# nadongjun/mirbft

Hardware: AMD Instinct MI355X
Metric: SHA-256 digests/s (request + batch digests), Actions.Hash stream (higher is better)
Workload: dtype u32

## Files before the change

### mirbft_amd/csrc/mirsha_api.hip

```cpp
#include "mirsha_ctx.h"

namespace mirsha_api {

int fail(mirsha_ctx* c, int code, const char* fmt, ...) {
    char buf[512];
    va_list ap;
    va_start(ap, fmt);
    vsnprintf(buf, sizeof(buf), fmt, ap);
    va_end(ap);
    if (c) c->err = buf;
    return code;
}

hipEvent_t take_event(KernelTimer& t) {
    if (!t.pool.empty()) {
        hipEvent_t e = t.pool.back();
        t.pool.pop_back();
        return e;
    }
    hipEvent_t e = nullptr;
    if (hipEventCreate(&e) != hipSuccess) return nullptr;
    return e;
}

// ... 81 lines not shown

int queue_bucket_order(mirsha_ctx* c, const OrderShape& sh, const uint32_t* d_len, uint32_t n, uint32_t* d_order) {
    uint32_t* counts = c->d_order_counts.as<uint32_t>();
    const size_t cells = (size_t)sh.bins * sh.n_chunks;
    uint32_t* base = counts + cells;
    if (int rc = timed_launch(c, kTimerOrder, [&] {
            return mirsha::launch_order_count(d_len, n, sh.bmax, sh.bins, sh.chunk, sh.n_chunks, counts, c->stream);
        }))
        return rc;
    size_t scan_bytes = sh.scan_bytes;
    HIP_TRY(c, mirsha::launch_counts_scan(c->d_scan.p, scan_bytes, counts, base, cells, c->stream));
    return timed_launch(c, kTimerOrder, [&] {
        return mirsha::launch_order_scatter(d_len, n, sh.bmax, sh.bins, sh.chunk, sh.n_chunks, base, d_order,
                                            c->stream);
    });
}

}

extern "C" {

int mirsha_version(void) { return (0 << 16) | 2; }

int mirsha_device_count(int* count) {
    if (!count) return MIRSHA_EINVAL;
    int n = 0;
    if (hipGetDeviceCount(&n) != hipSuccess) {
        (void)hipGetLastError();
        n = 0;
    }
    *count = n;
    return MIRSHA_OK;
}

int mirsha_ctx_create(int device, mirsha_ctx** out) {
    if (!out) return MIRSHA_EINVAL;
    *out = nullptr;
    int n = 0;
    if (hipGetDeviceCount(&n) != hipSuccess || n <= 0) {
        (void)hipGetLastError();
        return MIRSHA_ENODEV;
    }
    if (device < 0 || device >= n) return MIRSHA_EINVAL;
    hipDeviceProp_t prop;
    if (hipGetDeviceProperties(&prop, device) != hipSuccess) return MIRSHA_EHIP;
    if (strncmp(prop.gcnArchName, "gfx950", 6) != 0) return MIRSHA_ENODEV;
    mirsha_ctx* c = new mirsha_ctx();
    c->device = device;
    if (hipSetDevice(device) != hipSuccess || hipStreamCreateWithFlags(&c->own, hipStreamNonBlocking) != hipSuccess) {
        delete c;
        return MIRSHA_EHIP;
    }
    c->stream = c->own;
    *out = c;
    return MIRSHA_OK;
}

void mirsha_ctx_destroy(mirsha_ctx* c) {
    if (!c) return;
    (void)hipSetDevice(c->device);
    (void)hipStreamSynchronize(c->stream);
    if (c->xin) (void)hipStreamSynchronize(c->xin);
    if (c->xout) (void)hipStreamSynchronize(c->xout);
    if (c->xcommit) (void)hipStreamSynchronize(c->xcommit);
    for (auto& t : c->timers) {
        for (auto& pr : t.pending) { (void)hipEventDestroy(pr.first); (void)hipEventDestroy(pr.second); }
        for (auto e : t.pool) (void)hipEventDestroy(e);
    }
    c->d_arena.release(); c->d_off.release(); c->d_len.release(); c->d_order.release();
    c->d_out.release(); c->d_idx.release(); c->d_first.release(); c->d_out2.release(); c->d_scratch.release();
    c->d_scan.release();
    c->d_order_counts.release();
    for (int k = 0; k < kStageSlots; k++) {
        c->h_ring[k].release();
        if (c->ring_ev[k]) (void)hipEventDestroy(c->ring_ev[k]);
    }
    c->h_meta.release();
    c->h_outs.release();
    c->d_meta.release();
    c->h_expect.release(); c->h_verdict.release(); c->d_expect.release(); c->d_verdict.release();
    for (auto e : c->xev) (void)hipEventDestroy(e);
    if (c->xin) (void)hipStreamDestroy(c->xin);
    if (c->xout) (void)hipStreamDestroy(c->xout);
    if (c->xcommit) (void)hipStreamDestroy(c->xcommit);
    for (auto& sl : c->slots) {
        sl.stage.release(); sl.dig.release(); sl.dev.release(); sl.stage2.release(); sl.dev2.release();
        sl.xp.stage.release(); sl.xp.verdict.release(); sl.xp.dev.release();
        sl.cm.stage.release(); sl.cm.dev.release(); sl.cm.snap.release(); sl.cm.rows.release();
        if (sl.done) (void)hipEventDestroy(sl.done);
        if (sl.ev_in) (void)hipEventDestroy(sl.ev_in);
        if (sl.ev_kern) (void)hipEventDestroy(sl.ev_kern);
    }
    if (c->own) (void)hipStreamDestroy(c->own);
    delete c;
}

const char* mirsha_last_error(const mirsha_ctx* c) { return c ? c->err.c_str() : "null context"; }

int mirsha_ctx_set_stream(mirsha_ctx* c, void* s) {
    if (!c) return MIRSHA_EINVAL;
    c->stream = s ? static_cast<hipStream_t>(s) : c->own;
    return MIRSHA_OK;
}

void* mirsha_ctx_stream(mirsha_ctx* c) { return c ? static_cast<void*>(c->stream) : nullptr; }

int mirsha_ctx_set_variant(mirsha_ctx* c, int v) {
    if (!c || !mirsha::variant_valid(v)) return MIRSHA_EINVAL;
    c->variant = v;
    return MIRSHA_OK;
}

int mirsha_ctx_set_timing(mirsha_ctx* c, int enable) {
    if (!c) return MIRSHA_EINVAL;
    c->timing = enable != 0;
    return MIRSHA_OK;
}

int mirsha_ctx_kernel_time(mirsha_ctx* c, int which, uint64_t* launches, double* total_ms) {
    if (!c || which < 0 || which >= kKernelTimers) return MIRSHA_EINVAL;
    if (int rc = use_device(c)) return rc;
    KernelTimer& t = c->timers[which];
    for (auto& pr : t.pending) {
        HIP_TRY(c, hipEventSynchronize(pr.second));
// ... 237 lines not shown
```

### mirbft_amd/csrc/mirsha_ctx.h

```cpp
#pragma once
#include <hip/hip_runtime.h>

#include <algorithm>
#include <atomic>
#include <chrono>
#include <condition_variable>
#include <cstdarg>
#include <cstdio>
#include <cstdlib>
#include <cstring>
#include <functional>
#include <mutex>
#include <string>
#include <thread>
#include <vector>

#include "../../include/mirsha.h"
#include "mirsha_host.h"
#include "mirsha_device.h"
#include "mirsha_order.h"
#include "mirsha_sha512.h"
#include "mirsha_sha512_pair.h"
#include "mirsha_sha512_plan.h"

// ... 107 lines not shown
    uint8_t* out = nullptr;
    uint32_t n = 0;
    uint64_t* bits = nullptr;
    uint32_t* count = nullptr;
};

struct AsyncSlot {
    PinnedBuf stage;
    Clock::time_point t_queued;
    PinnedBuf dig;
    DevBuf dev;
    PinnedBuf stage2;
    DevBuf dev2;
    hipEvent_t done = nullptr;
    hipEvent_t ev_in = nullptr, ev_kern = nullptr;
    uint64_t ticket = 0;
    bool busy = false;
    SlotRetire retire;
    std::vector<uint32_t> rank;
    double prof[MIRSHA_PROF_PHASES] = {};
    ExpectSlot xp;
    CommitSlot cm;
};

constexpr int kKernelTimers = 10;
constexpr int kTimerVerify = 6;
constexpr int kTimerExpect = 7;
constexpr int kTimerOrder = 8;
constexpr int kTimerStreams = 9;

struct KernelTimer {
    std::vector<std::pair<hipEvent_t, hipEvent_t>> pending;
    std::vector<hipEvent_t> pool;
    uint64_t launches = 0;
    double ms = 0.0;
};


}
using namespace mirsha_api;

struct mirsha_ctx {
    int device = 0;
    hipStream_t own = nullptr;
    hipStream_t stream = nullptr;
    int variant = mirsha::kVariantLds;
    int hasher = MIRSHA_HASHER_SHA256;
    mutable uint64_t sha512_pair_launches = 0;
    bool timing = false;
    uint32_t time_mask = 0xFFFFFFFFu;
    std::string err;
    DevBuf d_arena, d_off, d_len, d_order, d_out, d_idx, d_first, d_out2, d_scratch;
    DevBuf d_scan;
    int order_mode = MIRSHA_ORDER_HOST;
    DevBuf d_order_counts;
    PinnedBuf h_ring[kStageSlots];
    hipEvent_t ring_ev[kStageSlots] = {};
    bool ring_busy[kStageSlots] = {};
    PinnedBuf h_meta, h_outs;
    DevBuf d_meta;
    hipStream_t xin = nullptr, xout = nullptr;
    std::vector<hipEvent_t> xev;
    std::vector<uint32_t> sl_len;
    std::vector<uint64_t> sl_poff;
    KernelTimer timers[kKernelTimers];
    PinnedBuf h_expect, h_verdict;
    DevBuf d_expect, d_verdict;
    AsyncSlot slots[kAsyncSlots];
    std::vector<uint64_t> xp_has;
    std::vector<uint32_t> xp_base;
    hipStream_t xcommit = nullptr;
    std::vector<uint32_t> cm_plan;
    uint64_t next_ticket = 1;
    uint64_t done_ticket = 0;
    double prof[MIRSHA_PROF_PHASES] = {};
};

struct RingOwner {
    hipEvent_t ev = nullptr;
    bool queued = false;
};

struct mirsha_chains {
    int device = 0;
    uint32_t n = 0;
    int hasher = MIRSHA_HASHER_SHA256;
    DevBuf d_h, d_pend, d_cnt;
    DevBuf d_dig, d_pos, d_act, d_afirst, d_which, d_out;
    std::vector<uint32_t> plan;
    DevBuf d_plan;
    RingOwner ring;
    uint64_t pair_launches = 0;
};

struct mirsha_streams {
    int device = 0;
    uint32_t n = 0;
    int hasher = MIRSHA_HASHER_SHA256;
    uint32_t row_bytes = 0;
    DevBuf d_state;
    std::vector<uint32_t> act, efirst, kind, len;
    std::vector<uint64_t> off, poff;
    std::vector<uint32_t> seg_stream, sfirst, seg_flags;
    PinnedBuf stage;
    DevBuf dev, d_out;
    RingOwner ring;
// ... 22 lines not shown
    DevBuf d_seg_nb, d_seg_state, d_seg_flags;
    uint64_t seg_runs = 0;
    int fallback = 0;
    uint32_t test_placement = 0;
    DevBuf d_probe;
    bool trace = false;
    std::vector<uint32_t> cidx, cfirst;
    uint32_t uniform = 0;
    std::vector<uint32_t> order;
    DevBuf d_cidx, d_cfirst, d_order;
};

namespace mirsha_api {

int fail(mirsha_ctx* c, int code, const char* fmt, ...);

#define HIP_TRY(c, expr)                                                                    \
    do {                                                                                    \
        hipError_t _e = (expr);                                                             \
        if (_e != hipSuccess)                                                               \
            return fail((c), _e == hipErrorOutOfMemory ? MIRSHA_ENOMEM : MIRSHA_EHIP,       \
                        "%s: %s (%s:%d)", #expr, hipGetErrorString(_e), __FILE__, __LINE__); \
    } while (0)

hipEvent_t take_event(KernelTimer& t);

template <class F>
int timed_launch(mirsha_ctx* c, int which, F&& launch) {
    hipEvent_t e0 = nullptr, e1 = nullptr;
    const bool timed = c->timing && ((c->time_mask >> which) & 1u);
    if (timed) {
        e0 = take_event(c->timers[which]);
        e1 = take_event(c->timers[which]);
        if (e0 && e1) mirsha::next_launch_events() = {e0, e1};
    }
    hipError_t e = launch();
    const bool bound = e0 && e1 && !mirsha::next_launch_events().start;
    mirsha::next_launch_events() = {};
    if (timed && (!bound || e != hipSuccess)) {
        if (e0) c->timers[which].pool.push_back(e0);
        if (e1) c->timers[which].pool.push_back(e1);
    }
    if (e != hipSuccess) return fail(c, MIRSHA_EHIP, "kernel launch: %s", hipGetErrorString(e));
    if (bound) c->timers[which].pending.emplace_back(e0, e1);
    return MIRSHA_OK;
}

inline hipError_t hasher_launch_msgs(const mirsha_ctx* c, const uint8_t* arena, uint64_t arena_len,
                                     const uint64_t* off, const uint32_t* len, const uint32_t* order, uint32_t n,
                                     uint8_t* out, hipStream_t s) {
    if (c->hasher == MIRSHA_HASHER_SHA512_256)
        return mirsha::launch_sha512_msgs(arena, arena_len, off, len, order, n, out, c->variant, s,
                                          &c->sha512_pair_launches);
    return mirsha::launch_msgs(arena, arena_len, off, len, order, n, out, c->variant, s);
}
inline hipError_t hasher_launch_lists(const mirsha_ctx* c, const uint8_t* digests, uint32_t n_digests,
                                      const uint32_t* idx, uint32_t n_entries, const uint32_t* first, uint32_t n_lists,
                                      uint32_t* scratch, uint8_t* out, hipStream_t s) {
    if (c->hasher == MIRSHA_HASHER_SHA512_256)
        return mirsha::launch_sha512_lists(digests, n_digests, idx, n_entries, first, n_lists, scratch, out, s,
                                           &c->sha512_pair_launches);
    return mirsha::launch_lists(digests, n_digests, idx, n_entries, first, n_lists, scratch, out, s);
}

inline const char* hasher_name(int hasher) { return hasher == MIRSHA_HASHER_SHA512_256 ? "sha512_256" : "sha256"; }

inline int sha256_only(mirsha_ctx* c, const char* call) {
    if (!c || c->hasher == MIRSHA_HASHER_SHA256) return MIRSHA_OK;
    return fail(c, MIRSHA_EINVAL, "%s: hasher %s is not built for this call", call, hasher_name(c->hasher));
}

inline int chains_hasher_match(mirsha_ctx* c, const mirsha_chains* ch, const char* call) {
    if (!c || !ch || c->hasher == ch->hasher) return MIRSHA_OK;
    return fail(c, MIRSHA_EINVAL, "%s: the chains hash with %s, the context with %s", call, hasher_name(ch->hasher),
                hasher_name(c->hasher));
}

inline int plan_hasher_match(mirsha_ctx* c, const mirsha_pipeline* p, const char* call) {
    if (!c || !p || c->hasher == p->hasher) return MIRSHA_OK;
    return fail(c, MIRSHA_EINVAL, "%s: the plan hashes with %s, the context with %s", call, hasher_name(p->hasher),
                hasher_name(c->hasher));
}

inline int streams_hasher_match(mirsha_ctx* c, const mirsha_streams* st, const char* call) {
    if (!c || !st || c->hasher == st->hasher) return MIRSHA_OK;
    return fail(c, MIRSHA_EINVAL, "%s: the streams hash with %s, the context with %s", call, hasher_name(st->hasher),
                hasher_name(c->hasher));
}

int use_device(mirsha_ctx* c);

inline uint32_t host_blocks(uint32_t L) { return (uint32_t)(((uint64_t)L + 72u) >> 6); }

bool bucket_order(const uint32_t* len, uint32_t n, uint32_t* order);

struct OrderShape {
    uint32_t bmax = 0, bins = 0, chunk = 0, n_chunks = 0;
    size_t scan_bytes = 0;
};
int order_buffers(mirsha_ctx* c, uint32_t n, uint32_t bmin, uint32_t bmax, OrderShape* shape);
int queue_bucket_order(mirsha_ctx* c, const OrderShape& shape, const uint32_t* d_len, uint32_t n, uint32_t* d_order);

inline int owner_order(mirsha_ctx* c, const RingOwner& o) {
    if (!o.queued) return MIRSHA_OK;
    HIP_TRY(c, hipStreamWaitEvent(c->stream, o.ev, 0));
    return MIRSHA_OK;
}
// ... 210 lines not shown
```

### mirbft_amd/csrc/mirsha_kernels.h

```cpp
#pragma once
#include <hip/hip_runtime.h>
#include <stdint.h>

namespace mirsha {

constexpr uint32_t kWavesPerBlock = 4;
constexpr uint32_t kBlockThreads = 64 * kWavesPerBlock;
constexpr uint32_t kNullIndex = 0xFFFFFFFFu;

enum : int {
    kVariantLds = 0,
    kVariantDirect = 1,
    kVariantLowOcc = 4,
    kVariantLdsOnly = 5,
    kVariantPair = 6,
    kVariantCu = 10,
};
const char* ab_getenv(const char* name);
inline bool variant_valid(int v) {
    return v == kVariantLds || v == kVariantDirect || v == kVariantLowOcc || v == kVariantLdsOnly || v == kVariantPair ||
           v == kVariantCu;
}
constexpr uint32_t kCuMaxWavesPerSimd = 4;
uint32_t cu_count();
constexpr uint32_t kLowOccTiles = 1024;
constexpr uint32_t kPairMaxGroups = 512;
uint32_t pair_max_groups();

constexpr uint64_t kMaxBufferArena = 0xFFFFFF00ull;
constexpr uint32_t kMaxBufferMsgs = 1u << 27;
hipError_t launch_offsets_scan(void* tmp, size_t& tmp_bytes, const uint32_t* len, uint64_t* off, uint32_t n,
                               hipStream_t s);
struct LaunchEvents {
    hipEvent_t start = nullptr, stop = nullptr;
};
LaunchEvents& next_launch_events();

hipError_t launch_msgs(const uint8_t* arena, uint64_t arena_len, const uint64_t* off,
                       const uint32_t* len, const uint32_t* order, uint32_t n, uint8_t* out,
                       int variant, hipStream_t s);
constexpr uint32_t kMaxListDigests = (1u << 27) - 1u;
constexpr uint32_t kMaxListEntries = (1u << 30) - 1u;
hipError_t launch_lists(const uint8_t* digests, uint32_t n_digests, const uint32_t* idx, uint32_t n_entries,
                        const uint32_t* first, uint32_t n_lists, uint32_t* scratch, uint8_t* out, hipStream_t s);
struct PadBlockKW {
    uint32_t kw[64];
    uint32_t use;
};
PadBlockKW pad_block_kw(uint64_t L);
hipError_t launch_chain(const uint8_t* digests, uint32_t n_digests, const uint32_t* cidx, uint32_t n_entries,
                        const uint32_t* cfirst, uint32_t n_lists, uint8_t* out, hipStream_t s, uint32_t uniform = 0);
hipError_t launch_chain_pair(const uint8_t* digests, uint32_t n_digests, const uint32_t* cidx, uint32_t n_entries,
                             const uint32_t* cfirst, uint32_t n_lists, uint8_t* out, hipStream_t s);
struct OverlapArgs {
    const uint8_t* arena;
    uint64_t arena_len;
    const uint64_t* off;
    const uint32_t* len;
    const uint32_t* order;
    uint32_t n_req;
    uint8_t* req_out;
    const uint8_t* prev_digests;
    uint32_t n_req_prev;
    const uint32_t* cidx;
    uint32_t n_entries;
    const uint32_t* cfirst;
    uint32_t n_lists;
    uint8_t* list_out;
    uint32_t list_waves;
    uint32_t chain_prio;
};
hipError_t launch_msgs_overlap(const OverlapArgs& a, hipStream_t s);
constexpr uint32_t kFusedChunkBlocks = 2;
constexpr uint32_t kFusedMaxQueues = 4;
constexpr uint32_t kCtlTileTicket = 0, kCtlDone = 80, kCtlWords = 96;
constexpr unsigned long long kFusedWatchdogTicks = 200000000ull;
struct FusedArgs {
    const uint8_t* arena;
    const uint64_t* off;
    const uint32_t* len;
    const uint32_t* order;
    uint8_t* req_out;
    const uint32_t* cidx;
    const uint32_t* cfirst;
    uint8_t* list_out;
    const uint32_t* tadj_first;
    const uint32_t* tadj;
    const uint32_t* cbase;
    const uint32_t* expected;
    unsigned long long* counters;
    unsigned long long* ctl;
    unsigned long long* err;
    unsigned long long watchdog;
// ... 43 lines not shown
```

### mirbft_amd/csrc/mirsha_kernels.hip

```cpp
#include <algorithm>
#include <atomic>
#include <cstdlib>
#include <cstdio>
#include <type_traits>

#include "mirsha_device.h"

namespace mirsha {

struct RawChunk {
    uint32_t v[5];
    uint32_t sel;
};

__device__ __forceinline__ void issue_chunk(__amdgpu_buffer_rsrc_t rsrc, uint32_t records, uint32_t o,
                                            uint32_t blk, uint32_t q, bool active, RawChunk& c) {
    const uint32_t addr = o + 64u * blk + 16u * q;
    const uint32_t a = active ? (addr & ~3u) : 0xFFFFFFE0u;
    c.sel = be_sel(addr & 3u);
    if (a + 20u <= records || !active) {
        const auto v = __builtin_amdgcn_raw_buffer_load_b128(rsrc, a, 0, 0);
        c.v[0] = v[0]; c.v[1] = v[1]; c.v[2] = v[2]; c.v[3] = v[3];
        c.v[4] = __builtin_amdgcn_raw_buffer_load_b32(rsrc, a + 16u, 0, 0);
    } else {
// ... 161 lines not shown
__device__ __forceinline__ void balance_done() {
    __hip_atomic_store(g_bal_prog + bal_word(), kBalDone, __ATOMIC_RELAXED, __HIP_MEMORY_SCOPE_WORKGROUP);
}

__device__ __forceinline__ void wave_lds_handoff() {
    __builtin_amdgcn_fence(__ATOMIC_RELEASE, "wavefront");
    __builtin_amdgcn_wave_barrier();
    __builtin_amdgcn_fence(__ATOMIC_ACQUIRE, "wavefront");
}

__device__ __forceinline__ void tile_read_words(const uint4* tile, uint32_t lane, uint32_t w[16]) {
#pragma unroll
    for (int k = 0; k < 4; k++) {
        const uint4 x = tile[lds_slot(lane, (uint32_t)k)];
        w[4 * k + 0] = x.x; w[4 * k + 1] = x.y; w[4 * k + 2] = x.z; w[4 * k + 3] = x.w;
    }
}

__device__ __forceinline__ bool last_block_opaque(uint32_t wave_nb, uint32_t blk) {
    uint32_t wnb;
    asm volatile("s_mov_b32 %0, %1" : "=s"(wnb) : "s"(wave_nb));
    return wnb - blk == 1u;
}

template <bool kFused, bool kBuf>
__device__ __forceinline__ void tile_store(uint8_t* out, uint32_t n, uint32_t msg, const uint32_t st[8]) {
    if constexpr (kFused || kBuf) {
        const __amdgpu_buffer_rsrc_t ors =
            __builtin_amdgcn_make_buffer_rsrc((void*)out, (short)0, (int)(32u * n), 0x00020000);
        if constexpr (kFused)
            store_digest_sc1(ors, msg, st);
        else
            store_digest_buf(ors, msg, st);
    } else {
        store_digest(out, msg, st);
    }
}

template <bool kFused>
__device__ __forceinline__ void block_prio(uint32_t fprio, uint32_t blk) {
    if constexpr (kFused) {
        if (fprio == kPrioBalance)
            balance_prio(blk);
        else if (fprio == kPrioProgress)
            progress_prio(blk);
        else
            fixed_prio(fprio);
    } else {
        progress_prio(blk);
    }
}

constexpr uint32_t kTilePaused = 0, kTileDone = 1;
template <bool kLds, bool kWide, bool kFused = false, bool kDma = false>
__device__ __forceinline__ uint32_t hash_tile(const uint8_t* __restrict__ arena, uint64_t arena_len,
                                          const uint64_t* __restrict__ off, const uint32_t* __restrict__ len,
                                          const uint32_t* __restrict__ order, uint32_t n, uint8_t* __restrict__ out,
                                          uint4* my, uint32_t t, uint32_t lane, uint32_t fprio = 0,
                                          uint32_t b0 = 0u, uint32_t b1 = 0xFFFFFFFFu, uint32_t* st_io = nullptr,
                                          uint32_t lone_sel = 0u, uint4* my2 = nullptr,
                                          unsigned long long* lone_tr = nullptr) {
    __builtin_amdgcn_s_setprio(3);
    const uint32_t slot = t * 64u + lane;
    const bool valid = slot < n;
    const uint32_t slot_c = valid ? slot : n - 1u;
    const uint32_t msg = order ? order[slot_c] : slot_c;
    const uint32_t L_ = len[msg];
    const uint64_t o_ = off[msg];
    const uint32_t L = valid ? L_ : 0u;
    const uint64_t o = valid ? o_ : 0u;
    const uint32_t nb = valid ? blocks_for_len(L) : 0u;
    const uint32_t max_l = wave_max(valid ? L : 0u);
    const uint32_t wave_nb = blocks_for_len(max_l);

    const uint64_t records = (arena_len + 3u) & ~3ull;
    const __amdgpu_buffer_rsrc_t rsrc =
        __builtin_amdgcn_make_buffer_rsrc((void*)arena, (short)0, (int)(uint32_t)records, 0x00020000);
    auto issue = [&](uint64_t mo, uint32_t blk, uint32_t q, bool active, RawChunk& rc) {
        if constexpr (kWide)
            issue_chunk_wide(arena, records, mo, blk, q, active, rc);
        else
            issue_chunk(rsrc, (uint32_t)records, (uint32_t)mo, blk, q, active, rc);
    };

    uint32_t st[8];
#pragma unroll
    for (int i = 0; i < 8; i++) st[i] = (st_io && b0) ? st_io[i] : kH0[i];
    const bool finished = b1 >= wave_nb;

    if constexpr (kLds && !kWide) {
        const uint32_t q = lane & 3u;
        const uint64_t reach = valid ? o + 64ull * wave_nb + 20u : 0ull;
        const bool far = __builtin_amdgcn_ballot_w64(reach > records) == 0;
        const bool aligned = __builtin_amdgcn_ballot_w64(valid && (o & 3u) != 0u) == 0;
        const uint32_t min_l = wave_min(valid ? L : 0xFFFFFFFFu);
        const bool uni = max_l == min_l;
        const int32_t u_last = (int32_t)(min_l - 64u * (wave_nb - 1u));
        const bool tail_ok = uni && u_last <= 16;
        const TailWords tw = tail_words(u_last, min_l);
        uint32_t vo[4], sel[4];
#pragma unroll
        for (int j = 0; j < 4; j++) {
            const uint32_t a = (uint32_t)__shfl((int)(uint32_t)o, 16 * j + (int)(lane >> 2), 64) + 16u * q;
            vo[j] = a & ~3u;
            sel[j] = be_sel(a & 3u);
        }
        auto stage = [&](uint32_t blk, uint32_t w[16], uint32_t ln, bool trim) {
            const uint32_t soff = 64u * blk;
            const uint32_t qq = ln & 3u;
            const bool skip = trim && soff + 16u * qq >= min_l;
            RawChunk rc[4];
            if (far && !trim) {
#pragma unroll
                for (int j = 0; j < 4; j++) {
                    const auto v = __builtin_amdgcn_raw_buffer_load_b128(rsrc, vo[j], soff, 0);
                    rc[j].v[0] = v[0]; rc[j].v[1] = v[1]; rc[j].v[2] = v[2]; rc[j].v[3] = v[3];
                    rc[j].v[4] = 0u;
                }
                if (!aligned) {
#pragma unroll
                    for (int j = 0; j < 4; j++)
                        rc[j].v[4] = __builtin_amdgcn_raw_buffer_load_b32(rsrc, vo[j], soff + 16u, 0);
                }
            } else if (far) {
#pragma unroll
                for (int j = 0; j < 4; j++) {
                    const uint32_t a = skip ? 0xFFFFFFE0u : vo[j] + soff;
                    const auto v = __builtin_amdgcn_raw_buffer_load_b128(rsrc, a, 0, 0);
                    rc[j].v[0] = v[0]; rc[j].v[1] = v[1]; rc[j].v[2] = v[2]; rc[j].v[3] = v[3];
                    rc[j].v[4] = aligned ? 0u : __builtin_amdgcn_raw_buffer_load_b32(rsrc, a + 16u, 0, 0);
                }
            } else {
#pragma unroll
                for (int j = 0; j < 4; j++)
                    issue_chunk(rsrc, (uint32_t)records, vo[j] + soff, 0u, 0u, !skip, rc[j]);
            }
            const bool pad = soff + 64u > min_l;
#pragma unroll
            for (int j = 0; j < 4; j++) {
                uint32_t wq[4];
#pragma unroll
                for (int k = 0; k < 4; k++) wq[k] = be_word(rc[j].v[k + 1], rc[j].v[k], sel[j]);
                if (pad && !uni) {
                    const uint32_t Lm = (uint32_t)__shfl((int)L, 16 * j + (int)(ln >> 2), 64);
                    pad_words(soff + 16u * qq, Lm, blk + 1u == blocks_for_len(Lm), qq, wq);
                }
                my[lds_slot(16u * j + (ln >> 2), qq)] = make_uint4(wq[0], wq[1], wq[2], wq[3]);
            }
            wave_lds_handoff();
            tile_read_words(my, ln, w);
            wave_lds_handoff();
        };
// ... 33 lines not shown
                uint32_t w[16];
                const uint4* tb = tile_of(blk);
#pragma unroll
                for (int k = 0; k < 4; k++) {
                    const uint4 x = tb[lds_slot(lane, (uint32_t)k)];
                    w[4 * k + 0] = x.x; w[4 * k + 1] = x.y; w[4 * k + 2] = x.z; w[4 * k + 3] = x.w;
                }
                asm volatile("s_waitcnt lgkmcnt(0)" ::: "memory");
                if (blk + (deep ? 2u : 1u) < d1) issue_dma(blk + (deep ? 2u : 1u));
#pragma unroll
                for (int k = 0; k < 16; k++) w[k] = __builtin_bswap32(w[k]);
                if (soff + 64u > dmin) {
                    const bool last = last_block_opaque(wave_nb, blk);
                    if (uni) {
                        pad_block_uniform(w, soff, dmin, last);
                    } else {
#pragma unroll
                        for (int k = 0; k < 4; k++)
                            pad_words(soff + 16u * (uint32_t)k, L, blk + 1u == nb, (uint32_t)k, &w[4 * k]);
                    }
                }
                if constexpr (!kFused) block_prio<false>(fprio, blk);
                if constexpr (kFused) {
                    if (lone_sel != 0u && simd_alone(lone_sel)) lone_sel = kLoneSeen;
                    if (lone_sel == kLoneSeen) {
                        if (lone_tr != nullptr) {
                            if (lane == 0u) *lone_tr |= 1ull << 63 | (unsigned long long)min(blk, 1023u) << 53;
                            lone_tr = nullptr;
                        }
                        if (blk < nb) compress_asm_lat(st, w);
                    } else if (blk < nb) {
                        compress_asm(st, w);
                    }
                } else if (blk < nb) {
                    compress_asm(st, w);
                }
            }
        }
        for (uint32_t blk = dma ? loop_end : b0; blk < loop_end; blk++) {
            const uint32_t soff = 64u * blk;
            uint32_t w[16];
            stage(blk, w, lane, false);
            if (soff + 64u > min_l && uni)
                pad_block_uniform(w, soff, min_l, last_block_opaque(wave_nb, blk));
            block_prio<kFused>(fprio, blk);
            if (blk < nb) compress_asm(st, w);
        }
        if (tail_ok && finished) {
            const uint32_t blk = wave_nb - 1u;
            uint32_t w[16];
            uint32_t ln;
            asm volatile("v_mov_b32 %0, %1" : "=v"(ln) : "v"(lane));
            stage(blk, w, ln, true);
            pad_block_uniform<4>(w, 64u * blk, min_l, false);
            block_prio<kFused>(fprio, blk);
            if (blk < nb) compress_asm_tail(st, w, tw);
        }
    } else if constexpr (kLds) {
        const uint32_t q = lane & 3u;
        uint32_t Lj[4], nbj[4];
        uint64_t oj[4];
#pragma unroll
        for (int j = 0; j < 4; j++) {
            const int src = 16 * j + (int)(lane >> 2);
            Lj[j] = (uint32_t)__shfl((int)L, src, 64);
            oj[j] = (uint64_t)(uint32_t)__shfl((int)(uint32_t)o, src, 64);
            oj[j] |= (uint64_t)(uint32_t)__shfl((int)(uint32_t)(o >> 32), src, 64) << 32;
            nbj[j] = (uint32_t)__shfl((int)nb, src, 64);
        }
        for (uint32_t blk = 0; blk < wave_nb; blk++) {
            RawChunk rc[4];
#pragma unroll
            for (int j = 0; j < 4; j++) issue(oj[j], blk, q, blk < nbj[j], rc[j]);
#pragma unroll
            for (int j = 0; j < 4; j++) {
                uint32_t wq[4];
                finish_chunk(rc[j], 64u * blk + 16u * q, Lj[j], blk + 1u == nbj[j], q, wq);
                my[lds_slot(16u * j + (lane >> 2), q)] = make_uint4(wq[0], wq[1], wq[2], wq[3]);
            }
            wave_lds_handoff();
            uint32_t w[16];
#pragma unroll
            for (int k = 0; k < 4; k++) {
                const uint4 x = my[lds_slot(lane, (uint32_t)k)];
                w[4 * k + 0] = x.x; w[4 * k + 1] = x.y; w[4 * k + 2] = x.z; w[4 * k + 3] = x.w;
            }
            wave_lds_handoff();
            progress_prio(blk);
            if (blk < nb) compress_asm(st, w);
        }
    } else {
        for (uint32_t blk = 0; blk < wave_nb; blk++) {
            const bool active = blk < nb;
            RawChunk rc[4];
#pragma unroll
            for (int q = 0; q < 4; q++) issue(o, blk, (uint32_t)q, active, rc[q]);
            uint32_t w[16];
#pragma unroll
            for (int q = 0; q < 4; q++)
                finish_chunk(rc[q], 64u * blk + 16u * q, L, blk + 1u == nb, (uint32_t)q, &w[4 * q]);
            progress_prio(blk);
            if (active) compress_asm(st, w);
        }
    }
    if (!finished) {
#pragma unroll
        for (int i = 0; i < 8; i++) st_io[i] = st[i];
        return kTilePaused;
    }
    if (valid) tile_store<kFused, kLds && !kWide>(out, n, msg, st);
    return kTileDone;
}

constexpr uint32_t kMsgWaves = 1;
constexpr uint32_t kMsgOcc = 8, kTileSlots = 256;
template <bool kLds, bool kWide = false>
__global__ __launch_bounds__(64 * kMsgWaves, kWide ? 6 : kMsgOcc) void sha256_msgs_kernel(
    const uint8_t* __restrict__ arena, uint64_t arena_len, const uint64_t* __restrict__ off,
    const uint32_t* __restrict__ len, const uint32_t* __restrict__ order, uint32_t n,
    uint8_t* __restrict__ out) {
    __shared__ uint4 tile[kMsgWaves][kTileSlots];
    const uint32_t lane = threadIdx.x & 63u;
    const uint32_t wv = threadIdx.x >> 6;
    const uint32_t t = blockIdx.x * kMsgWaves + wv;
    if (t * 64u >= n) return;
    hash_tile<kLds, kWide>(arena, arena_len, off, len, order, n, out, tile[wv], t, lane);
}

constexpr uint32_t kCuLds = 96u * 1024u;
__global__ __launch_bounds__(1024, 1) void sha256_msgs_cu_kernel(const uint8_t* __restrict__ arena,
                                                                 uint64_t arena_len,
                                                                 const uint64_t* __restrict__ off,
                                                                 const uint32_t* __restrict__ len,
                                                                 const uint32_t* __restrict__ order, uint32_t n,
                                                                 uint8_t* __restrict__ out) {
    extern __shared__ uint4 cu_lds[];
    const uint32_t lane = threadIdx.x & 63u;
    const uint32_t wv = threadIdx.x >> 6;
    const uint32_t t = blockIdx.x * (blockDim.x >> 6) + wv;
    if (t * 64u >= n) return;
    hash_tile<true, false, false, true>(arena, arena_len, off, len, order, n, out, cu_lds + 256u * wv, t, lane);
}

__device__ __forceinline__ void overlap_chain(const uint8_t* __restrict__ digests, uint32_t n_digests,
                                              const uint32_t* __restrict__ cidx, uint32_t n_entries,
                                              const uint32_t* __restrict__ cfirst, uint32_t n_lists,
                                              uint8_t* __restrict__ list_out, uint32_t g, uint32_t lane,
                                              uint32_t prio_mode) {
    __builtin_amdgcn_s_setprio(3);
    const uint32_t k = g * 64u + lane;
    const bool valid = k < n_lists;
    const uint32_t kc = valid ? k : n_lists - 1u;
    const uint32_t e0_ = cfirst[kc], e1_ = cfirst[kc + 1];
    const uint32_t e0 = valid ? e0_ : 0u;
    const uint32_t c = valid ? e1_ - e0_ : 0u;
    const uint32_t L = 32u * c;
    const uint32_t nb = valid ? blocks_for_len(L) : 0u;
    const uint32_t wave_nb = blocks_for_len(32u * wave_max(c));
    const __amdgpu_buffer_rsrc_t drs = buffer_rsrc(digests, 32u * n_digests);
    const __amdgpu_buffer_rsrc_t irs = buffer_rsrc(cidx, 4u * n_entries);
    uint32_t st[8];
#pragma unroll
    for (int i = 0; i < 8; i++) st[i] = kH0[i];
    uint32_t i0 = ld_u32(irs, 4u * e0, 0u < c), i1 = ld_u32(irs, 4u * (e0 + 1u), 1u < c);
    for (uint32_t blk = 0; blk < wave_nb; blk++) {
        const uint32_t d0 = 2u * blk;
        uint4 x[4];
        load_digest(drs, i0, d0 < c, x[0], x[1]);
        load_digest(drs, i1, d0 + 1u < c, x[2], x[3]);
        i0 = ld_u32(irs, 4u * (e0 + d0 + 2u), d0 + 2u < c);
        i1 = ld_u32(irs, 4u * (e0 + d0 + 3u), d0 + 3u < c);
        uint32_t w[16];
        list_block_words(x, d0, c, w);
        if (blk + 1u == nb) list_block_length(w, L);
        fixed_prio(prio_mode == 0u   ? 3u - min(3u, 4u * blk / wave_nb)
                   : prio_mode == 1u ? 3u - min(3u, blk)
                   : prio_mode == 2u ? 3u
                                     : 1u);
        if (blk < nb) compress_asm(st, w);
// ... 844 lines not shown
}

hipError_t launch_clock_probe(uint32_t blocks, uint32_t iters, unsigned long long* stamps, uint32_t* sink,
                              hipStream_t s) {
    launch_k(clock_probe_kernel, blocks, 256, 0, s, iters, stamps, sink);
    return hipGetLastError();
}


const char* ab_getenv(const char* name) {
    const char* ab = getenv("MIRSHA_AB");
    return (ab && ab[0] == '1') ? getenv(name) : nullptr;
}

uint32_t pair_max_groups() {
    static const uint32_t v = [] {
        if ((getenv("MIRSHA_PAIR") || getenv("MIRSHA_PAIR_MAX_GROUPS")) && !ab_getenv("MIRSHA_PAIR_MAX_GROUPS") &&
            !ab_getenv("MIRSHA_PAIR"))
            fprintf(stderr, "mirsha: MIRSHA_PAIR / MIRSHA_PAIR_MAX_GROUPS are A/B knobs, read only with MIRSHA_AB=1; "
                            "ignored\n");
        const char* e = ab_getenv("MIRSHA_PAIR");
        if (e && e[0] == '0') return 0u;
        const char* m = ab_getenv("MIRSHA_PAIR_MAX_GROUPS");
        return m ? (uint32_t)strtoul(m, nullptr, 10) : kPairMaxGroups;
    }();
    return v;
}

uint32_t cu_count() {
    static std::atomic<uint32_t> cached[64] = {};
    int dev = 0;
    if (hipGetDevice(&dev) != hipSuccess || dev < 0 || dev >= 64) return 256u;
    uint32_t v = cached[dev].load(std::memory_order_relaxed);
    if (!v) {
        int a = 0;
        if (hipDeviceGetAttribute(&a, hipDeviceAttributeMultiprocessorCount, dev) != hipSuccess || a <= 0) a = 256;
        v = (uint32_t)a;
        cached[dev].store(v, std::memory_order_relaxed);
    }
    return v;
}

enum DynLdsKernel { kDynLdsCu, kDynLdsFused, kDynLdsProbe, kDynLdsKernels };
hipError_t dyn_lds_attr(const void* fn, DynLdsKernel form, uint32_t bytes) {
    static std::atomic<uint8_t> done[64][kDynLdsKernels] = {};
    int dev = 0;
    if (hipError_t e = hipGetDevice(&dev)) return e;
    if (dev >= 0 && dev < 64 && done[dev][form].load(std::memory_order_acquire)) return hipSuccess;
    if (hipError_t e = hipFuncSetAttribute(fn, hipFuncAttributeMaxDynamicSharedMemorySize, (int)bytes)) return e;
    if (dev >= 0 && dev < 64) done[dev][form].store(1, std::memory_order_release);
    return hipSuccess;
}

hipError_t launch_msgs(const uint8_t* arena, uint64_t arena_len, const uint64_t* off,
                       const uint32_t* len, const uint32_t* order, uint32_t n, uint8_t* out,
                       int variant, hipStream_t s) {
    if (n == 0) return hipSuccess;
    const uint32_t tiles = (n + 63u) / 64u;
    const uint32_t grid = (tiles + kWavesPerBlock - 1u) / kWavesPerBlock;
    const uint32_t mgrid = (tiles + kMsgWaves - 1u) / kMsgWaves;
    if (arena_len > kMaxBufferArena || n >= kMaxBufferMsgs) {
        launch_k(sha256_msgs_kernel<true, true>, mgrid, 64 * kMsgWaves, 0, s, arena, arena_len, off, len, order, n, out);
        return hipGetLastError();
    }
    if (variant == kVariantPair || (variant == kVariantLds && tiles <= pair_max_groups())) {
        launch_k(sha256_msgs_pair_kernel, tiles, kPairThreads, 0, s, arena, arena_len, off, len, order, n, out);
        return hipGetLastError();
    }
    if (variant == kVariantLowOcc || (variant == kVariantLds && tiles <= kLowOccTiles)) {
        launch_k(sha256_msgs_lowocc_kernel, grid, kBlockThreads, 0, s, arena, arena_len, off, len, order, n, out);
        return hipGetLastError();
    }
    if (variant == kVariantCu || (variant == kVariantLds && tiles <= kCuMaxWavesPerSimd * 4u * cu_count())) {
        const uint32_t k = (tiles + 4u * cu_count() - 1u) / (4u * cu_count());
        const uint32_t wg_waves = 4u * std::min(k, kCuMaxWavesPerSimd);
        const uint32_t cgrid = (tiles + wg_waves - 1u) / wg_waves;
        if (hipError_t e = dyn_lds_attr((const void*)sha256_msgs_cu_kernel, kDynLdsCu, kCuLds)) return e;
        launch_k(sha256_msgs_cu_kernel, cgrid, 64u * wg_waves, kCuLds, s, arena, arena_len, off, len, order, n, out);
        return hipGetLastError();
    }
    if (variant == kVariantDirect)
        launch_k(sha256_msgs_kernel<false>, mgrid, 64 * kMsgWaves, 0, s, arena, arena_len, off, len, order, n, out);
    else
        launch_k(sha256_msgs_kernel<true>, mgrid, 64 * kMsgWaves, 0, s, arena, arena_len, off, len, order, n, out);
    return hipGetLastError();
}

hipError_t launch_msgs_overlap(const OverlapArgs& a, hipStream_t s) {
    const uint32_t tiles = (a.n_req + 63u) / 64u;
    if (a.list_waves + tiles == 0) return hipSuccess;
    if (a.arena_len > kMaxBufferArena || a.n_req >= kMaxBufferMsgs || (a.list_waves && a.n_lists == 0))
        return hipErrorInvalidValue;
    launch_k(sha256_msgs_overlap_kernel, a.list_waves + tiles, 64, 0, s, a);
    return hipGetLastError();
}

hipError_t launch_lists(const uint8_t* digests, uint32_t n_digests, const uint32_t* idx, uint32_t n_entries,
                        const uint32_t* first, uint32_t n_lists, uint32_t* scratch, uint8_t* out, hipStream_t s) {
    if (n_lists == 0) return hipSuccess;
    const uint32_t grid = (n_lists + kBlockThreads - 1u) / kBlockThreads;
    launch_k(sha256_lists_kernel, grid, kBlockThreads, 0, s, digests, n_digests, idx, n_entries, first, n_lists, scratch,
                                                      out);
    return hipGetLastError();
}

PadBlockKW pad_block_kw(uint64_t L) {
    auto rotr = [](uint32_t x, int n) { return (x >> n) | (x << (32 - n)); };
    uint32_t w[64] = {0x80000000u};
    w[14] = (uint32_t)(L >> 29);
    w[15] = (uint32_t)(L << 3);
    for (int j = 16; j < 64; j++) {
        const uint32_t s0 = rotr(w[j - 15], 7) ^ rotr(w[j - 15], 18) ^ (w[j - 15] >> 3);
        const uint32_t s1 = rotr(w[j - 2], 17) ^ rotr(w[j - 2], 19) ^ (w[j - 2] >> 10);
        w[j] = w[j - 16] + s0 + w[j - 7] + s1;
    }
    PadBlockKW p{};
    for (int j = 0; j < 64; j++) p.kw[j] = kK[j] + w[j];
    p.use = 1u;
    return p;
}

hipError_t launch_chain(const uint8_t* digests, uint32_t n_digests, const uint32_t* cidx, uint32_t n_entries,
                        const uint32_t* cfirst, uint32_t n_lists, uint8_t* out, hipStream_t s, uint32_t uniform) {
    if (n_lists == 0) return hipSuccess;
    const uint32_t grid = (n_lists + kBlockThreads - 1u) / kBlockThreads;
    if (uniform) {
        if ((uint64_t)(n_lists - 1u) * uniform >= n_entries || (uint64_t)n_lists * uniform < n_entries)
            return hipErrorInvalidValue;
        PadBlockKW pad{};
        if ((uniform & 1u) == 0u) {
            pad = pad_block_kw(32ull * uniform);
            const char* e = ab_getenv("MIRSHA_CHAIN_PAD");
            pad.use = !(e && e[0] == '0');
        }
        launch_k(sha256_chain_kernel<true>, grid, kBlockThreads, 0, s, digests, n_digests, cidx, n_entries, cfirst,
                 n_lists, out, uniform, pad);
    } else {
// ... 83 lines not shown
```

### mirbft_amd/csrc/mirsha_plan.hip

```cpp
#include "mirsha_ctx.h"

namespace mirsha_api {

uint32_t uniform_lists(const std::vector<uint32_t>& cidx, const std::vector<uint32_t>& cfirst) {
    const size_t n_lists = cfirst.size() - 1, n = cidx.size();
    if (n_lists == 0 || n == 0 || cfirst[1] == 0) return 0;
    const uint64_t B = cfirst[1];
    if ((n_lists - 1) * B >= n || n_lists * B < n) return 0;
    for (size_t k = 0; k < n_lists; k++)
        if (cfirst[k] != k * B) return 0;
    for (size_t e = 0; e < n; e++)
        if (cidx[e] != e) return 0;
    if (const char* e = mirsha::ab_getenv("MIRSHA_CHAIN_UNIFORM"))
        if (e[0] == '0') return 0;
    return (uint32_t)B;
}

int pipeline_build(mirsha_ctx* c, mirsha_pipeline* p, uint32_t n_req, const uint32_t* idx, const uint32_t* first,
                   uint32_t n_lists, const uint32_t* len) {
    p->n_req = n_req;
    p->n_lists = n_lists;
    p->cfirst.assign(n_lists + 1, 0);
    p->cidx.clear();
    p->cidx.reserve(first[n_lists]);
    std::vector<uint8_t> listed(n_req, 0);
    for (uint32_t k = 0; k < n_lists; k++) {
        for (uint32_t e = first[k]; e < first[k + 1]; e++) {
            if (idx[e] == MIRSHA_NULL_INDEX) continue;
            p->cidx.push_back(idx[e]);
            listed[idx[e]] = 1;
        }
        p->cfirst[k + 1] = (uint32_t)p->cidx.size();
    }
    p->n_entries = (uint32_t)p->cidx.size();
    p->uniform = uniform_lists(p->cidx, p->cfirst);
    p->order.resize(n_req);
    for (uint32_t r = 0; r < n_req; r++) p->order[r] = r;
    std::stable_sort(p->order.begin(), p->order.end(), [&](uint32_t x, uint32_t y) {
        if (listed[x] != listed[y]) return listed[x] > listed[y];
        return len ? host_blocks(len[x]) > host_blocks(len[y]) : false;
    });
    HIP_TRY(c, p->d_cidx.ensure(sizeof(uint32_t) * std::max<uint32_t>(p->n_entries, 1)));
    HIP_TRY(c, p->d_cfirst.ensure(sizeof(uint32_t) * (n_lists + 1)));
    HIP_TRY(c, p->d_order.ensure(sizeof(uint32_t) * std::max<uint32_t>(n_req, 1)));
    if (p->n_entries)
        HIP_TRY(c, hipMemcpyAsync(p->d_cidx.p, p->cidx.data(), sizeof(uint32_t) * p->n_entries, hipMemcpyHostToDevice, c->stream));
    HIP_TRY(c, hipMemcpyAsync(p->d_cfirst.p, p->cfirst.data(), sizeof(uint32_t) * (n_lists + 1), hipMemcpyHostToDevice, c->stream));
    if (n_req)
        HIP_TRY(c, hipMemcpyAsync(p->d_order.p, p->order.data(), sizeof(uint32_t) * n_req, hipMemcpyHostToDevice, c->stream));
    HIP_TRY(c, hipStreamSynchronize(c->stream));
    return MIRSHA_OK;
}

struct PlanKernels {
    hipError_t (*requests)(const mirsha_ctx* c, const mirsha_pipeline* p, const uint8_t* d_arena, uint64_t arena_len,
                           const uint64_t* d_off, const uint32_t* d_len, uint8_t* d_req_out);
    hipError_t (*lists)(const mirsha_ctx* c, const mirsha_pipeline* p, const uint8_t* d_digests, uint8_t* d_list_out);
    hipError_t (*overlap)(const mirsha_ctx* c, const mirsha_pipeline* p, bool tiles, bool chains,
                          const uint8_t* d_arena, uint64_t arena_len, const uint64_t* d_off, const uint32_t* d_len,
                          uint8_t* d_req_out, const uint8_t* d_prev_req, uint8_t* d_prev_batch_out);
};

const PlanKernels kPlanSha256 = {
    [](const mirsha_ctx* c, const mirsha_pipeline* p, const uint8_t* d_arena, uint64_t arena_len, const uint64_t* d_off,
       const uint32_t* d_len, uint8_t* d_req_out) {
        return mirsha::launch_msgs(d_arena, arena_len, d_off, d_len, p->d_order.as<uint32_t>(), p->n_req, d_req_out,
                                   c->variant, c->stream);
    },
    [](const mirsha_ctx* c, const mirsha_pipeline* p, const uint8_t* d_digests, uint8_t* d_list_out) {
        if ((p->n_lists + 63u) / 64u <= mirsha::pair_max_groups())
            return mirsha::launch_chain_pair(d_digests, p->n_req, p->d_cidx.as<uint32_t>(), p->n_entries,
                                             p->d_cfirst.as<uint32_t>(), p->n_lists, d_list_out, c->stream);
        return mirsha::launch_chain(d_digests, p->n_req, p->d_cidx.as<uint32_t>(), p->n_entries,
                                    p->d_cfirst.as<uint32_t>(), p->n_lists, d_list_out, c->stream, p->uniform);
    },
    [](const mirsha_ctx* c, const mirsha_pipeline* p, bool tiles, bool chains, const uint8_t* d_arena,
       uint64_t arena_len, const uint64_t* d_off, const uint32_t* d_len, uint8_t* d_req_out, const uint8_t* d_prev_req,
       uint8_t* d_prev_batch_out) {
        mirsha::OverlapArgs a{};
        a.arena = d_arena;
        a.arena_len = tiles ? arena_len : 0;
        a.off = d_off;
        a.len = d_len;
        a.order = p->d_order.as<uint32_t>();
        a.n_req = tiles ? p->n_req : 0u;
        a.req_out = d_req_out;
        a.prev_digests = d_prev_req;
        a.n_req_prev = p->n_req;
        a.cidx = p->d_cidx.as<uint32_t>();
        a.n_entries = p->n_entries;
        a.cfirst = p->d_cfirst.as<uint32_t>();
        a.n_lists = p->n_lists;
        a.list_out = d_prev_batch_out;
        a.list_waves = chains ? (p->n_lists + 63u) / 64u : 0u;
        if (const char* e = mirsha::ab_getenv("MIRSHA_OVERLAP_CHAIN_PRIO")) a.chain_prio = (uint32_t)atoi(e) & 3u;
        return mirsha::launch_msgs_overlap(a, c->stream);
    },
};

const PlanKernels kPlanSha512 = {
    [](const mirsha_ctx* c, const mirsha_pipeline* p, const uint8_t* d_arena, uint64_t arena_len, const uint64_t* d_off,
       const uint32_t* d_len, uint8_t* d_req_out) {
        return mirsha::launch_sha512_msgs(d_arena, arena_len, d_off, d_len, p->d_order.as<uint32_t>(), p->n_req,
                                          d_req_out, c->variant, c->stream, &c->sha512_pair_launches);
    },
    [](const mirsha_ctx* c, const mirsha_pipeline* p, const uint8_t* d_digests, uint8_t* d_list_out) {
        return mirsha::launch_sha512_plan_lists(d_digests, p->n_req, p->d_cidx.as<uint32_t>(), p->n_entries,
                                                p->d_cfirst.as<uint32_t>(), p->n_lists, p->uniform, d_list_out,
                                                c->stream, &c->sha512_pair_launches);
    },
    [](const mirsha_ctx* c, const mirsha_pipeline* p, bool tiles, bool chains, const uint8_t* d_arena,
       uint64_t arena_len, const uint64_t* d_off, const uint32_t* d_len, uint8_t* d_req_out, const uint8_t* d_prev_req,
       uint8_t* d_prev_batch_out) {
        mirsha::Sha512OverlapArgs a{};
        a.arena = d_arena;
        a.arena_len = tiles ? arena_len : 0;
        a.off = d_off;
        a.len = d_len;
        a.order = p->d_order.as<uint32_t>();
        a.n_req = tiles ? p->n_req : 0u;
// ... 525 lines not shown
```

Baseline: 5.110 billion.

## Make SHA-256 message kernel persistent with sharded atomic tile tickets

The default LDS message kernel now launches a fixed number of resident workgroups (occupancy times CUs times four) instead of one per tile. Each workgroup claims further tiles from one of up to 16 sharded global atomic counters and resets its counter after the last claim. Per-tile tail words are recomputed inside the block loop, and kernel arguments are reread from the kernarg segment to keep register pressure down. The aim is to cut launch and wave-dispatch overhead and balance uneven tiles, at the cost of atomic traffic, a small device control buffer per context, and reliance on correct counter resets between launches.

Result: slower. 4.867 billion (-4.8%).

```diff
diff --git a/mirbft_amd/csrc/mirsha_api.hip b/mirbft_amd/csrc/mirsha_api.hip
--- a/mirbft_amd/csrc/mirsha_api.hip
+++ b/mirbft_amd/csrc/mirsha_api.hip
@@ -157,6 +157,12 @@
         return MIRSHA_EHIP;
     }
     c->stream = c->own;
+    if (hipMalloc((void**)&c->d_msgs_ctl, mirsha::kMsgsCtlBytes) != hipSuccess ||
+        hipMemsetAsync(c->d_msgs_ctl, 0, mirsha::kMsgsCtlBytes, c->own) != hipSuccess ||
+        hipStreamSynchronize(c->own) != hipSuccess) {
+        mirsha_ctx_destroy(c);
+        return MIRSHA_EHIP;
+    }
     *out = c;
     return MIRSHA_OK;
 }
@@ -175,6 +181,7 @@
     c->d_arena.release(); c->d_off.release(); c->d_len.release(); c->d_order.release();
     c->d_out.release(); c->d_idx.release(); c->d_first.release(); c->d_out2.release(); c->d_scratch.release();
     c->d_scan.release();
+    if (c->d_msgs_ctl) (void)hipFree(c->d_msgs_ctl);
     c->d_order_counts.release();
     for (int k = 0; k < kStageSlots; k++) {
         c->h_ring[k].release();
diff --git a/mirbft_amd/csrc/mirsha_ctx.h b/mirbft_amd/csrc/mirsha_ctx.h
--- a/mirbft_amd/csrc/mirsha_ctx.h
+++ b/mirbft_amd/csrc/mirsha_ctx.h
@@ -183,6 +183,7 @@
     std::string err;
     DevBuf d_arena, d_off, d_len, d_order, d_out, d_idx, d_first, d_out2, d_scratch;
     DevBuf d_scan;
+    unsigned long long* d_msgs_ctl = nullptr;
     int order_mode = MIRSHA_ORDER_HOST;
     DevBuf d_order_counts;
     PinnedBuf h_ring[kStageSlots];
@@ -311,7 +312,7 @@
     if (c->hasher == MIRSHA_HASHER_SHA512_256)
         return mirsha::launch_sha512_msgs(arena, arena_len, off, len, order, n, out, c->variant, s,
                                           &c->sha512_pair_launches);
-    return mirsha::launch_msgs(arena, arena_len, off, len, order, n, out, c->variant, s);
+    return mirsha::launch_msgs(arena, arena_len, off, len, order, n, out, c->variant, s, c->d_msgs_ctl);
 }
 inline hipError_t hasher_launch_lists(const mirsha_ctx* c, const uint8_t* digests, uint32_t n_digests,
                                       const uint32_t* idx, uint32_t n_entries, const uint32_t* first, uint32_t n_lists,
diff --git a/mirbft_amd/csrc/mirsha_kernels.h b/mirbft_amd/csrc/mirsha_kernels.h
--- a/mirbft_amd/csrc/mirsha_kernels.h
+++ b/mirbft_amd/csrc/mirsha_kernels.h
@@ -36,9 +36,10 @@
 };
 LaunchEvents& next_launch_events();
 
+constexpr size_t kMsgsCtlBytes = 16 * 128;
 hipError_t launch_msgs(const uint8_t* arena, uint64_t arena_len, const uint64_t* off,
                        const uint32_t* len, const uint32_t* order, uint32_t n, uint8_t* out,
-                       int variant, hipStream_t s);
+                       int variant, hipStream_t s, unsigned long long* ctl);
 constexpr uint32_t kMaxListDigests = (1u << 27) - 1u;
 constexpr uint32_t kMaxListEntries = (1u << 30) - 1u;
 hipError_t launch_lists(const uint8_t* digests, uint32_t n_digests, const uint32_t* idx, uint32_t n_entries,
diff --git a/mirbft_amd/csrc/mirsha_kernels.hip b/mirbft_amd/csrc/mirsha_kernels.hip
--- a/mirbft_amd/csrc/mirsha_kernels.hip
+++ b/mirbft_amd/csrc/mirsha_kernels.hip
@@ -237,7 +237,7 @@
 }
 
 constexpr uint32_t kTilePaused = 0, kTileDone = 1;
-template <bool kLds, bool kWide, bool kFused = false, bool kDma = false>
+template <bool kLds, bool kWide, bool kFused = false, bool kDma = false, bool kRes = false>
 __device__ __forceinline__ uint32_t hash_tile(const uint8_t* __restrict__ arena, uint64_t arena_len,
                                           const uint64_t* __restrict__ off, const uint32_t* __restrict__ len,
                                           const uint32_t* __restrict__ order, uint32_t n, uint8_t* __restrict__ out,
@@ -282,7 +282,8 @@
         const bool uni = max_l == min_l;
         const int32_t u_last = (int32_t)(min_l - 64u * (wave_nb - 1u));
         const bool tail_ok = uni && u_last <= 16;
-        const TailWords tw = tail_words(u_last, min_l);
+        TailWords tw = {};
+        if constexpr (!kRes) tw = tail_words(u_last, min_l);
         uint32_t vo[4], sel[4];
 #pragma unroll
         for (int j = 0; j < 4; j++) {
@@ -422,6 +423,11 @@
             uint32_t ln;
             asm volatile("v_mov_b32 %0, %1" : "=v"(ln) : "v"(lane));
             stage(blk, w, ln, true);
+            if constexpr (kRes) {
+                uint32_t ml;
+                asm volatile("s_mov_b32 %0, %1" : "=s"(ml) : "s"(min_l));
+                tw = tail_words((int32_t)(ml - 64u * blk), ml);
+            }
             pad_block_uniform<4>(w, 64u * blk, min_l, false);
             block_prio<kFused>(fprio, blk);
             if (blk < nb) compress_asm_tail(st, w, tw);
@@ -478,23 +484,80 @@
         for (int i = 0; i < 8; i++) st_io[i] = st[i];
         return kTilePaused;
     }
+    if constexpr (kRes) {
+#pragma unroll
+        for (int i = 0; i < 8; i++) st_io[i] = st[i];
+        return kTileDone;
+    }
     if (valid) tile_store<kFused, kLds && !kWide>(out, n, msg, st);
     return kTileDone;
 }
 
 constexpr uint32_t kMsgWaves = 1;
 constexpr uint32_t kMsgOcc = 8, kTileSlots = 256;
+struct ResidentArgs {
+    unsigned long long* ctl;
+    uint32_t tiles;
+    uint32_t waves;
+    uint32_t shift;
+};
+constexpr uint32_t kResShardsLog2 = 4;
 template <bool kLds, bool kWide = false>
 __global__ __launch_bounds__(64 * kMsgWaves, kWide ? 6 : kMsgOcc) void sha256_msgs_kernel(
     const uint8_t* __restrict__ arena, uint64_t arena_len, const uint64_t* __restrict__ off,
     const uint32_t* __restrict__ len, const uint32_t* __restrict__ order, uint32_t n,
-    uint8_t* __restrict__ out) {
+    uint8_t* __restrict__ out, ResidentArgs res) {
     __shared__ uint4 tile[kMsgWaves][kTileSlots];
     const uint32_t lane = threadIdx.x & 63u;
     const uint32_t wv = threadIdx.x >> 6;
-    const uint32_t t = blockIdx.x * kMsgWaves + wv;
+    uint32_t t = blockIdx.x * kMsgWaves + wv;
     if (t * 64u >= n) return;
-    hash_tile<kLds, kWide>(arena, arena_len, off, len, order, n, out, tile[wv], t, lane);
+    if constexpr (kLds && !kWide) {
+        (void)lane;
+        static_assert(kMsgWaves == 1, "one ticket per workgroup");
+        t = blockIdx.x;
+        struct Args {
+            const uint8_t* arena; uint64_t arena_len; const uint64_t* off; const uint32_t* len;
+            const uint32_t* order; uint32_t n; uint8_t* out; ResidentArgs res;
+        };
+        const __attribute__((address_space(4))) Args* ka =
+            (const __attribute__((address_space(4))) Args*)__builtin_amdgcn_kernarg_segment_ptr();
+        uint32_t tiles;
+        do {
+            asm volatile("" : "+s"(ka));
+            uint32_t ln;
+            asm volatile("v_mbcnt_lo_u32_b32 %0, -1, 0\n\tv_mbcnt_hi_u32_b32 %0, -1, %0" : "=v"(ln));
+            uint32_t st[8];
+            hash_tile<true, false, false, false, true>(
+                ka->arena, ka->arena_len, ka->off, ka->len, ka->order, ka->n, nullptr, tile[wv], t, ln, 0u, 0u,
+                0xFFFFFFFFu, st);
+            asm volatile("" : "+s"(ka));
+            asm volatile("v_mbcnt_lo_u32_b32 %0, -1, 0\n\tv_mbcnt_hi_u32_b32 %0, -1, %0" : "=v"(ln));
+            const uint32_t n_ = ka->n;
+            tiles = ka->res.tiles;
+            const uint32_t waves = ka->res.waves, shift = ka->res.shift;
+            const uint32_t shard = blockIdx.x & ((1u << shift) - 1u);
+            const uint32_t shard_tiles = (tiles - waves + (1u << shift) - 1u - shard) >> shift;
+            const uint32_t shard_claims = shard_tiles + ((waves + (1u << shift) - 1u - shard) >> shift);
+            unsigned long long* ctr = ka->res.ctl + 16u * shard;
+            uint32_t tk = 0;
+            if (ln == 0u)
+                tk = (uint32_t)__hip_atomic_fetch_add(ctr, 1ull, __ATOMIC_RELAXED, __HIP_MEMORY_SCOPE_AGENT);
+            uint32_t ts;
+            asm volatile("s_mov_b32 %0, %1" : "=s"(ts) : "s"(t));
+            const uint32_t slot = ts * 64u + ln;
+            if (slot < n_) {
+                const uint32_t* order = ka->order;
+                tile_store<false, true>(ka->out, n_, order ? order[slot] : slot, st);
+            }
+            const uint32_t c = (uint32_t)__builtin_amdgcn_readfirstlane((int)tk);
+            if (c + 1u == shard_claims && ln == 0u)
+                __hip_atomic_store(ctr, 0ull, __ATOMIC_RELAXED, __HIP_MEMORY_SCOPE_AGENT);
+            t = c < shard_tiles ? waves + shard + (c << shift) : tiles;
+        } while (t < tiles);
+    } else {
+        hash_tile<kLds, kWide>(arena, arena_len, off, len, order, n, out, tile[wv], t, lane);
+    }
 }
 
 constexpr uint32_t kCuLds = 96u * 1024u;
@@ -1445,15 +1508,24 @@
     return hipSuccess;
 }
 
+uint32_t resident_slots() {
+    static const uint32_t knob = [] {
+        const char* e = ab_getenv("MIRSHA_RESIDENT_SLOTS");
+        return e ? (uint32_t)strtoul(e, nullptr, 10) : 0u;
+    }();
+    return knob ? knob : kMsgOcc * 4u * cu_count();
+}
+
 hipError_t launch_msgs(const uint8_t* arena, uint64_t arena_len, const uint64_t* off,
                        const uint32_t* len, const uint32_t* order, uint32_t n, uint8_t* out,
-                       int variant, hipStream_t s) {
+                       int variant, hipStream_t s, unsigned long long* ctl) {
     if (n == 0) return hipSuccess;
     const uint32_t tiles = (n + 63u) / 64u;
     const uint32_t grid = (tiles + kWavesPerBlock - 1u) / kWavesPerBlock;
     const uint32_t mgrid = (tiles + kMsgWaves - 1u) / kMsgWaves;
     if (arena_len > kMaxBufferArena || n >= kMaxBufferMsgs) {
-        launch_k(sha256_msgs_kernel<true, true>, mgrid, 64 * kMsgWaves, 0, s, arena, arena_len, off, len, order, n, out);
+        launch_k(sha256_msgs_kernel<true, true>, mgrid, 64 * kMsgWaves, 0, s, arena, arena_len, off, len, order, n, out,
+                 ResidentArgs{});
         return hipGetLastError();
     }
     if (variant == kVariantPair || (variant == kVariantLds && tiles <= pair_max_groups())) {
@@ -1472,10 +1544,17 @@
         launch_k(sha256_msgs_cu_kernel, cgrid, 64u * wg_waves, kCuLds, s, arena, arena_len, off, len, order, n, out);
         return hipGetLastError();
     }
-    if (variant == kVariantDirect)
-        launch_k(sha256_msgs_kernel<false>, mgrid, 64 * kMsgWaves, 0, s, arena, arena_len, off, len, order, n, out);
-    else
-        launch_k(sha256_msgs_kernel<true>, mgrid, 64 * kMsgWaves, 0, s, arena, arena_len, off, len, order, n, out);
+    if (variant == kVariantDirect) {
+        launch_k(sha256_msgs_kernel<false>, mgrid, 64 * kMsgWaves, 0, s, arena, arena_len, off, len, order, n, out,
+                 ResidentArgs{});
+        return hipGetLastError();
+    }
+    if (!ctl) return hipErrorInvalidValue;
+    const uint32_t waves = std::min(tiles, resident_slots());
+    uint32_t shift = 0;
+    while (shift < kResShardsLog2 && (2u << shift) <= waves) shift++;
+    const ResidentArgs res{ctl, tiles, waves, shift};
+    launch_k(sha256_msgs_kernel<true>, waves, 64 * kMsgWaves, 0, s, arena, arena_len, off, len, order, n, out, res);
     return hipGetLastError();
 }
 
diff --git a/mirbft_amd/csrc/mirsha_plan.hip b/mirbft_amd/csrc/mirsha_plan.hip
--- a/mirbft_amd/csrc/mirsha_plan.hip
+++ b/mirbft_amd/csrc/mirsha_plan.hip
@@ -65,7 +65,7 @@
     [](const mirsha_ctx* c, const mirsha_pipeline* p, const uint8_t* d_arena, uint64_t arena_len, const uint64_t* d_off,
        const uint32_t* d_len, uint8_t* d_req_out) {
         return mirsha::launch_msgs(d_arena, arena_len, d_off, d_len, p->d_order.as<uint32_t>(), p->n_req, d_req_out,
-                                   c->variant, c->stream);
+                                   c->variant, c->stream, c->d_msgs_ctl);
     },
     [](const mirsha_ctx* c, const mirsha_pipeline* p, const uint8_t* d_digests, uint8_t* d_list_out) {
         if ((p->n_lists + 63u) / 64u <= mirsha::pair_max_groups())
```
